# Unrepentant-Atheist/AC-3-ACM-Codec

Measured on AMD Instinct MI355X. Metric: AC-3 5.1@48kHz frames/sec/GPU (decode+encode); achieved HBM GB/s vs peak, higher is better.
Workload: dtype f32+i32

## Files before the change

ac-3-acm-codec_amd/csrc/decode.hip:

```cpp
#include "decode_kernel.h"

namespace ac3mi {

__global__ void lfsr_prefix_kernel(const uint32_t *draws, uint16_t *frame_lfsr, uint32_t *frame_pos, uint16_t *lfsr_state, const int32_t *slot,
                                   const uint16_t *seq, const uint16_t *idx, int n_streams, int frames)
{
    const int s = blockIdx.x * blockDim.x + threadIdx.x;
    if (s >= n_streams) return;
    uint32_t state = lfsr_state[slot ? slot[s] : s];
    uint32_t pos = idx[state];
    for (int f = 0; f < frames; f++) {
        if (frame_pos) frame_pos[(size_t)s * frames + f] = state ? pos : 0xffffffffu;
        else frame_lfsr[(size_t)s * frames + f] = (uint16_t)state;
        const uint32_t k = draws[(size_t)s * frames + f];
        if (state != 0 && k) { pos = (pos + k) % 65535u; state = seq[pos]; }
    }
    if (frame_pos) lfsr_state[slot ? slot[s] : s] = (uint16_t)state;
}

struct MantLDS {
    uint4 dsc[M2_NDESC];
    float qtab[760];
    uint8_t ring[6][M2_LDS_WAVE];
    uint8_t cplbnd[6][20];
};

#ifndef MANT_LB
#define MANT_LB 7
#endif
__global__ __launch_bounds__(384, MANT_LB) void mant_kernel(const MantParams P)
{
    __shared__ MantLDS L;
    extern __shared__ uint32_t frw[];
    const int tid = threadIdx.x, lane = tid & 63;
    const int blk = __builtin_amdgcn_readfirstlane(tid >> 6);
    const unsigned fidx = xcd_remap(blockIdx.x, gridDim.x);
    const size_t unit = (size_t)fidx * 6 + blk;
    const uint4 *dq = reinterpret_cast<const uint4 *>(P.desc + unit);
    const BlkWords D{{dq[0], dq[1], dq[2], dq[3], dq[4]}};
    const uint32_t fposv = P.frame_pos[fidx];
    const int nw = (P.frame_bytes + 3) >> 2;
    const auto fw = stage_frame_fetch<384>(P.frames + (size_t)fidx * P.frame_stride, P.frame_bytes, tid);
    const float q0 = P.tab->qtab[tid];
    float q1 = 0.f;
    if (tid < 760 - 384) q1 = P.tab->qtab[384 + tid];
    float *cblk = P.coef + unit * P.n_in * 256;
    MantBlk B;
    B.nf = P.nfchans; B.lfeon = P.lfeon; B.acmod = P.acmod; B.in_lfe = P.lfeon ? 1 : 0;
    const bool failed = D.head(B);
    const uint64_t rve = D.rv_exp(), rvb = D.rv_bap();
    const uint8_t *const rowbase = P.rows + (size_t)fidx * 6 * ROWSET;
    const RowFetch fetch{rowbase, rve, rvb, lane};
    {
        stage_frame_store<384>(frw, fw, P.frame_bytes, tid);
        if (const int own = D.own_bytes()) trim_staged_frame(frw, own, nw, tid, 384);
        if (tid < M2_NDESC) L.dsc[tid] = mant_desc2((uint32_t)tid);
        L.qtab[tid] = q0;
        if (tid < 760 - 384) L.qtab[384 + tid] = q1;
    }
    const int slot0 = seg_slot(0, B.nf, B.chincpl, B.chincpl ? __builtin_ctz(B.chincpl) : 99);
    uint2 first = make_uint2(0u, 0u);
    if (!failed) first = fetch(slot0);
    __syncthreads();
    if (failed) {
        for (int c = 0; c < P.n_in; c++)
            *reinterpret_cast<float4 *>(cblk + (size_t)c * 256 + 4 * lane) = make_float4(0.f, 0.f, 0.f, 0.f);
        return;
    }
    D.ranges(B);
    B.gainv = D.gainv(lane);
    if (B.chincpl && lane < 18) {
        const uint32_t below = D.cplbndstrc() & ((1u << lane) - 1u);
        L.cplbnd[blk][lane] = (uint8_t)(lane - __popc(below));
    }
    const uint32_t fpos = rfl(fposv);
    const bool lfsr_live = fpos != 0xffffffffu;
    const uint32_t i0 = lfsr_live ? (fpos + D.draw_off()) % 65535u : 0u;
    const float *cc = P.cplco + unit * 90;
    mant_block2<256, true>(B, fetch, first, [&](int c, int bnd) { return cc[c * 18 + bnd]; }, L.cplbnd[blk], L.dsc, L.ring[blk], frw, (uint32_t)nw + 2u,
                L.qtab, reinterpret_cast<const int16_t *>(P.lfsr_seq) + 1 + i0, lfsr_live, cblk, D.bitpos(), lane);
}

}

namespace ac3mi {

#ifdef DEC_STAMPS
}
extern "C" __attribute__((visibility("default"))) int ac3mi_debug_dec_cycles(unsigned long long *out8, int reset)
{
    if (hipMemcpyFromSymbol(out8, HIP_SYMBOL(ac3mi::g_dec_cycles), sizeof(unsigned long long) * 8) != hipSuccess) return -1;
    if (reset) { unsigned long long z[8] = {0}; if (hipMemcpyToSymbol(HIP_SYMBOL(ac3mi::g_dec_cycles), z, sizeof z) != hipSuccess) return -1; }
    return 0;
}
namespace ac3mi {
#endif

hipError_t launch_mantx(const DeviceTables &tab, const DecodeLaunch &L, const MantParams &M, const KernelLaunch &k, hipStream_t stream);
void launch_decode0_src(const DecodeParams &P, unsigned n_streams, size_t fr_bytes, hipStream_t stream);

hipError_t decode_params(const DeviceTables &tab, const DecodeLaunch &L, DecodeParams &P)
{
    if (L.frame_bytes > STAGE_MAX_BYTES) return hipErrorInvalidValue;
    const bool split = L.choice.split;
    P.desc = split ? (BlkDesc *)L.ws_desc : nullptr;
    P.rows = split ? L.ws_rows : nullptr;
    P.cplco = split ? L.ws_cplco : nullptr;
    P.frame_pos = split ? L.ws_fpos : nullptr;
    P.frames = L.frames;
    P.coef = L.coef;
    P.blksw = L.blksw;
    P.zs = L.zs;
    P.status = L.status;
    P.lfsr_state = L.lfsr;
    P.slot = L.slot;
    P.tap_exp = L.tap_exp;
    P.tap_bap = L.tap_bap;
    P.lfsr_seq = tab.lfsr_seq;
    P.lfsr_idx = tab.lfsr_idx;
    P.tab = tab.dec;
    P.n_streams = L.n_streams;
    P.frames_per_stream = L.frames_per_stream;
    P.frame_stride = L.frame_stride;
    P.frame_bytes = L.frame_bytes;
    P.req_flags = L.req_flags;
    P.level = L.level;
    P.dynrng_on = L.dynrng_on;
    P.acmod = L.acmod;
    P.lfeon = L.lfeon;
    P.nfchans = sync_nfchans(L.acmod & 7);
    P.n_in = P.nfchans + (L.lfeon ? 1 : 0);
    P.frame_draws = L.frame_draws;
    P.frame_lfsr = L.frame_lfsr;
    P.dyn_out = L.dyn_out;
    P.dyn_in = L.dyn_in;
    P.crc = L.crc;
    if (L.src_dyn) {
        if (L.dynrng_on || L.dyn_out || L.dyn_in) return hipErrorInvalidValue;
        P.src_dyn = L.src_dyn;
    }
    return hipSuccess;
}

template <uint32_t V> constexpr auto decode_variant()
{
    using Fn = void (*)(DecodeParams);
    if constexpr (V == V_SRC) return (Fn) nullptr;
    else return (Fn)decode_kernel<(int)(V & V_NUM), (V & V_FX) != 0, (V & V_SRC) != 0>;
}
template <uint32_t V> struct DecodeVariant { static constexpr auto fn = decode_variant<V>(); };

hipError_t launch_decode(const DeviceTables &tab, const DecodeLaunch &L, hipStream_t stream)
{
    DecodeParams P;
    const hipError_t ep = decode_params(tab, L, P);
    if (ep != hipSuccess) return ep;
    if (L.n_streams <= 0 || L.frames_per_stream <= 0) return hipSuccess;
    const DecChoice &c = L.choice;
    if (c.err || c.wg) return hipErrorInvalidValue;
    static const int lds_pad = getenv("AC3MI_DEC_LDS_PAD") ? atoi(getenv("AC3MI_DEC_LDS_PAD")) : 0;
    static const int mant_pad = getenv("AC3MI_MANT_LDS_PAD") ? atoi(getenv("AC3MI_MANT_LDS_PAD")) : 0;
    const size_t fr_bytes = staged_frame_lds(L.frame_bytes);
    for (int i = 0; i < c.n; i++) {
// ... 42 lines not shown
```

ac-3-acm-codec_amd/csrc/decode_kernel.h:

```cpp
#pragma once
#include "decode_common.h"
#include "mant2.h"

namespace ac3mi {


#ifndef DEC_LB0
#define DEC_LB0 4
#endif
#ifndef DEC_LBP
#define DEC_LBP 5
#endif
#ifdef DEC_STAMPS
__device__ unsigned long long g_dec_cycles[8];
#define DK_DECL() unsigned long long dk_t = 0, dk_acc[6] = {0, 0, 0, 0, 0, 0}
#define DK_T0() dk_t = __builtin_readcyclecounter()
#define DK_LAP(id) do { const unsigned long long t_ = __builtin_readcyclecounter(); dk_acc[id] += t_ - dk_t; dk_t = t_; } while (0)
#define DK_END() do { if (lane == 0) for (int i_ = 0; i_ < 6; i_++) atomicAdd(&g_dec_cycles[i_], dk_acc[i_]); } while (0)
#else
#define DK_DECL() do { } while (0)
#define DK_T0() do { } while (0)
#define DK_LAP(id) do { } while (0)
#define DK_END() do { } while (0)
#endif
// ... 341 lines not shown
                                const int mybai = st.cbai(slot);
                                const int mydeltbae = slot == 5 ? 2 : st.deltbae(slot == 6 ? 5 : slot);
                                const BaCtx c = ba_ctx(st.bai(), mybai, st.csnroffst(), st.halfrate(), L.hth,
                                                       mydeltbae == 2 ? nullptr : L.deltba[slot == 6 ? 5 : slot],
                                                       slot == 6 ? st.cplfleak() << 8 : 0, slot == 6 ? st.cplsleak() << 8 : 0);
                                bit_allocate_finish(L, L.bmask, c, slot == 6 ? st.cplstrtbnd() : 0, start, end, L.exp + row_off(slot), L.bap + row_off(slot), wide, h, lane);
                            }
                        }
#undef AC3MI_SLOT_END
                    }
                    wave_sync();
                }
                if (rd.get(1)) {
                    const int n = rd.get(9);
                    rd.skip(8 * n);
                }
            } while (0);

            if (!FX && P.tap_exp) {
                uint8_t *te = P.tap_exp + (fidx * 6 + blk) * 7 * 256;
                int8_t *tb = P.tap_bap + (fidx * 6 + blk) * 7 * 256;
                for (int c = 0; c < 7; c++)
                    for (int i = lane; i < 256; i += 64) {
                        const bool in = c != 5 || i < LFE_ROW;
                        te[c * 256 + i] = in ? L.exp[row_off(c) + i] : 0;
                        tb[c * 256 + i] = in ? unmap_width(L.bap[row_off(c) + i]) : 0;
                    }
            }

            if (!err) {
                DK_LAP(3);
                a52_downmix_coeff_hd(gain, acm, st.output, st.dynrng, st.clev, st.slev);

                if (!PARSE && st.chincpl && lane < 18) {
                    const uint32_t below = st.cplbndstrc & ((1u << lane) - 1u);
                    L.cplbnd[lane] = (uint8_t)(lane - __popc(below));
                }
                SegBase sb;
                sb.bit = rd.pos();
                sb.r3 = sb.r5 = sb.r11 = sb.draw = 0;
                if constexpr (!PARSE) {
                    MantBlk B;
                    B.nf = nf; B.lfeon = lfeon; B.acmod = acm; B.in_lfe = in_lfe;
                    B.chincpl = st.chincpl; B.dithmask = dithmask; B.rematflg = st.rematflg();
                    B.cplstrtmant = st.cplstrtmant; B.cplendmant = st.cplendmant();
#pragma unroll
                    for (int i = 0; i < 5; i++) { B.endmant[i] = st.endm(i); B.gain[i] = gain[i]; }
                    B.lfe_gain = (st.output & AC3MI_LFE) ? st.dynrng : 0.f;
                    const uint32_t lfsr_i0 = P.lfsr_idx[st.lfsr];
                    const bool lfsr_live = st.lfsr != 0;
                    mant_block<false>(B, [&](int slot) { return (const uint8_t *)L.exp + row_off(slot); },
                                          [&](int slot) { return (const int8_t *)L.bap + row_off(slot); },
                                          [&](int c, int bnd) { return L.cplco[c][bnd]; }, L.cplbnd, L.desc, L.gcode, frw, FB.last,
                                          P.tab->qtab, P.lfsr_seq, lfsr_i0, lfsr_live, cblk, sb, lane);
                    if (lfsr_live && sb.draw) st.lfsr = P.lfsr_seq[(lfsr_i0 + (uint32_t)sb.draw) % 65535u];
                } else {
                    const int cplfirst = st.chincpl ? __builtin_ctz(st.chincpl) : 99;
                    const int nseg = nf + (st.chincpl ? 1 : 0) + (lfeon ? 1 : 0);
                    const int ncpl_dith = __popc(st.chincpl & dithmask);
                    const int k = lane;
                    const int slot_l = st.chincpl ? (k <= cplfirst ? k : k == cplfirst + 1 ? 6 : k - 1 < nf ? k - 1 : 5) : (k < nf ? k : 5);
                    const bool seg_l = k < nseg;
                    const int end_l = (int)((uint32_t)(st.ends >> (8 * slot_l)) & 0xffu);
                    const int start_l = slot_l == 6 ? st.cplstrtmant : 0;
                    const int mult_l = slot_l < 5 ? (dithmask >> slot_l) & 1 : slot_l == 6 ? ncpl_dith : 0;
                    const uint32_t key_l = 0x80000000u | (uint32_t)start_l | ((uint32_t)end_l << 10);
                    uint32_t ca = L.tot[slot_l][0], cb = L.tot[slot_l][1];
                    for (unsigned long long miss = __ballot(seg_l && L.tot[slot_l][2] != key_l); miss; miss &= miss - 1) {
                        const int k0 = __builtin_ctzll(miss);
                        const int s0 = __builtin_amdgcn_readlane(slot_l, k0);
                        const RowTotals T = row_totals(L.bap + row_off(s0), __builtin_amdgcn_readlane(start_l, k0), __builtin_amdgcn_readlane(end_l, k0),
                                                       s0 == 5 ? LFE_ROW / 4 : 64, lane);
                        if (lane == k0) { ca = T.a; cb = T.b; L.tot[s0][0] = T.a; L.tot[s0][1] = T.b; L.tot[s0][2] = key_l; }
                    }
                    {
                        const uint32_t n3 = seg_l ? (ca >> 13) & 511u : 0u, n5 = seg_l ? ca >> 22 : 0u, n11 = seg_l ? cb & 511u : 0u;
                        const uint32_t nz = seg_l ? cb >> 9 : 0u, plain = seg_l ? ca & 0x1fffu : 0u;
                        const uint32_t own35 = n3 | (n5 << 16), p35 = wave_incl_scan_u32(own35) - own35, r11 = wave_incl_scan_u32(n11) - n11;
                        const uint32_t r3 = p35 & 0xffffu, r5 = p35 >> 16;
                        auto div3 = [](uint32_t x) { return (x * 0xaaabu) >> 17; };
                        const uint32_t o3 = div3(r3 + n3 + 2u) - div3(r3 + 2u), o5 = div3(r5 + n5 + 2u) - div3(r5 + 2u);
                        const uint32_t o11 = ((r11 + n11 + 1u) >> 1) - ((r11 + 1u) >> 1);
                        const uint32_t bits_l = plain + 5u * o3 + 7u * (o5 + o11);
                        const uint32_t tot = wave_sum_u32(bits_l | ((nz * (uint32_t)mult_l) << 16));
                        sb.bit += tot & 0xffffu;
                        sb.draw = (int)(tot >> 16);
                    }
                    {
                        uint8_t *rowset = P.rows + (fidx * 6 + blk) * (size_t)ROWSET;
                        const int used = ((1 << nf) - 1) | (lfeon ? 32 : 0) | (st.chincpl ? 64 : 0);
                        const int we = dirty_exp & used, wb = dirty_bap & used;
                        for (int m = we; m; m &= m - 1) {
                            const int s0 = __builtin_ctz(m);
                            if (lane < (s0 == 5 ? LFE_ROW / 4 : 64))
                                *reinterpret_cast<uint32_t *>(rowset + s0 * 512 + 4 * lane) = *reinterpret_cast<const uint32_t *>(L.exp + row_off(s0) + 4 * lane);
                        }
                        for (int m = wb; m; m &= m - 1) {
                            const int s0 = __builtin_ctz(m);
                            if (lane < (s0 == 5 ? LFE_ROW / 4 : 64))
                                *reinterpret_cast<uint32_t *>(rowset + s0 * 512 + 256 + 4 * lane) = *reinterpret_cast<const uint32_t *>(L.bap + row_off(s0) + 4 * lane);
                        }
                        dirty_exp &= ~we;
                        dirty_bap &= ~wb;
                        rv_exp = ((we >> lane) & 1) ? (uint32_t)blk : rv_exp;
                        rv_bap = ((wb >> lane) & 1) ? (uint32_t)blk : rv_bap;
                    }
                    if (st.chincpl) {
                        float *cc = P.cplco + (fidx * 6 + blk) * 90;
                        cc[lane] = (&L.cplco[0][0])[lane];
                        if (lane < 26) cc[64 + lane] = (&L.cplco[0][0])[64 + lane];
                    }
                    {
                        uint8_t *dp = reinterpret_cast<uint8_t *>(P.desc + (fidx * 6 + blk));
                        const uint32_t fl = ((uint32_t)st.chincpl << BLK_CHINCPL) | ((uint32_t)dithmask << BLK_DITH) | ((uint32_t)st.rematflg() << BLK_REMAT);
                        const uint32_t w0 = lane == 0 ? rd.pos() : lane == 1 ? frame_draws : lane == 2 ? fl : st.cplbndstrc;
                        if (lane < 4) reinterpret_cast<uint32_t *>(dp)[lane] = w0;
                        const int em = lane == 5 ? st.cplstrtmant : lane == 7 ? short_bytes : (int)((uint32_t)(st.ends >> (8 * (lane & 7))) & 0xffu);
                        if (lane < 8) reinterpret_cast<uint16_t *>(dp + offsetof(BlkDesc, endmant))[lane] = (uint16_t)em;
                        if (lane < 8) { dp[offsetof(BlkDesc, rv_exp) + lane] = (uint8_t)rv_exp; dp[offsetof(BlkDesc, rv_bap) + lane] = (uint8_t)rv_bap; }
                        const float gl = lane == 0 ? gain[0] : lane == 1 ? gain[1] : lane == 2 ? gain[2] : lane == 3 ? gain[3] : lane == 4 ? gain[4]
                                       : (st.output & AC3MI_LFE) ? st.dynrng : 0.f;
                        const uint32_t w12 = lane < 6 ? __float_as_uint(gl) : (uint32_t)(16 * st.csnroffst() + (st.cbai(0) >> 3));
                        if (lane < 7) reinterpret_cast<uint32_t *>(dp + offsetof(BlkDesc, gain))[lane] = w12;
                    }
                    bd_ok = true;
                }
                rd.seek(sb.bit);
                frame_draws += (uint32_t)sb.draw;
            }

            DK_LAP(4);
            if (err) { status |= 1u << blk; frame_dead = true; }
            if constexpr (PARSE) {
                if ((err || !bd_ok) && lane == 0) {
                    P.desc[fidx * 6 + blk].flags = BLK_FAILED;
                    P.desc[fidx * 6 + blk].src_snr = 0u;
                    P.desc[fidx * 6 + blk].own_bytes = (uint16_t)short_bytes;
                }
            }
            {
                if (err && !PARSE)
                    for (int c = 0; c < n_in; c++)
                        *reinterpret_cast<float4 *>(cblk + (size_t)c * 256 + 4 * lane) = make_float4(0.f, 0.f, 0.f, 0.f);
                if (P.blksw && lane < nfchans)
                    P.blksw[(fidx * 6 + blk) * nfchans + lane] = (uint8_t)(err ? 0 : ((blkswm >> lane) & 1));
            }
            __builtin_amdgcn_fence(__ATOMIC_RELEASE, "wavefront");
            __builtin_amdgcn_wave_barrier();
        }
        DK_LAP(5);
        if (const uint8_t *crcp = crc_verdicts()) {
            const uint32_t cv = crcp[fidx];
            if (!(status & 0x100u) || (cv & 0x40u)) status |= (cv & 3u) << 10;
        }
        if (lane == 0) P.status[fidx] = status | (reuse0 ? 0x200u : 0u);
        if (lane == 0 && P.zs) P.zs[fidx] = (uint8_t)((status & 0x100u) ? 0 : surround_level_is_zero(acm, st.output, st.slev));
        if (MODE == 5 && lane == 0) P.frame_draws[fidx] = frame_draws;
        if (MODE == 4) {
            if (lane == 0) P.frame_pos[fidx] = pos_live ? lfsr_pos : 0xffffffffu;
            lfsr_pos = (lfsr_pos + frame_draws) % 65535u;
        }
    }
    if (MODE == 0 && lane == 0) P.lfsr_state[sslot] = (uint16_t)st.lfsr;
    if (MODE == 4 && lane == 0 && pos_live) P.lfsr_state[sslot] = P.lfsr_seq[lfsr_pos];
    DK_END();
}

}
```

ac-3-acm-codec_amd/csrc/decode_mx.hip:

```cpp
#include <stdlib.h>
#include "mant2.h"
#include "xform_core.h"
#include "ac3mi_internal.h"

namespace ac3mi {

constexpr int MX_PLANE = 256 + 16;
constexpr int MX_WAVE = 6 * EX_GROUP * 8;
constexpr int MX_RING = 6 * MX_PLANE * 4;
constexpr int MX_TILE = 3072;
static_assert(MX_RING + M2_LDS_WAVE <= MX_WAVE && MX_TILE + 256 * 6 * 2 <= MX_WAVE && 48 * 8 * 8 <= MX_TILE, "region layout");

struct MantxParams {
    MantParams m;
    const uint8_t *blksw;
    float *delay;
    const int32_t *slot;
    int delay_stride;
    float *pcm;
    int16_t *pcm16;
    int8_t wslot[6];
    const float2 *tw_long, *tw_short;
    const float *window;
    float bias;
};

struct MantxLDS {
    uint4 dsc[M2_NDESC];
    float qtab[760];
    float2 tw[2][128];
    float win[256];
    uint8_t cplbnd[6][20];
    uint32_t ready[6];
    alignas(16) uint8_t wave[6][MX_WAVE];
};

#ifndef MANTX_LB
#define MANTX_LB 3
#endif
#ifdef MX_STAMPS
__device__ unsigned long long g_mx_cycles[6][8];
#define MX_T0() unsigned long long mx_t = __builtin_readcyclecounter()
#define MX_LAP(id) do { const unsigned long long t_ = __builtin_readcyclecounter(); if (lane == 0) atomicAdd(&g_mx_cycles[blk][id], t_ - mx_t); mx_t = t_; } while (0)
#else
#define MX_T0() do { } while (0)
#define MX_LAP(id) do { } while (0)
#endif
template <bool S16, bool FX = false>
__global__ __launch_bounds__(384, MANTX_LB) void mantx_kernel(const MantxParams Q)
{
    const MantParams &P = Q.m;
    const int n_in = FX ? 6 : P.n_in, nfchans = FX ? 5 : P.nfchans;
    __shared__ MantxLDS L;
    extern __shared__ uint32_t frw[];
    const int tid = threadIdx.x, lane = tid & 63;
    const int blk = __builtin_amdgcn_readfirstlane(tid >> 6);
    MX_T0();
    const unsigned fidx = xcd_remap(blockIdx.x, gridDim.x);
    const size_t unit = (size_t)fidx * 6 + blk;
    const uint4 *dq = reinterpret_cast<const uint4 *>(P.desc + unit);
    const BlkWords D{{dq[0], dq[1], dq[2], dq[3], dq[4]}};
    const uint32_t fposv = P.frame_pos[fidx];
    const int nw = (P.frame_bytes + 3) >> 2;
    static_assert(offsetof(MantxLDS, win) == offsetof(MantxLDS, tw) + sizeof(float2) * 256, "tw and win are one 3-KB stretch");
    const auto fw = stage_frame_fetch<384>(P.frames + (size_t)fidx * P.frame_stride, P.frame_bytes, tid);
    const float q0 = P.tab->qtab[tid];
    float q1 = 0.f;
    if (tid < 760 - 384) q1 = P.tab->qtab[384 + tid];
    const float2 *twsrc = blk < 2 ? Q.tw_long + tid : blk < 4 ? Q.tw_short + (tid - 128) : reinterpret_cast<const float2 *>(Q.window) + (tid - 256);
    const float2 twv = *twsrc;
    uint8_t *const region = L.wave[blk];
    float *const planes = reinterpret_cast<float *>(region);
    MantBlk B;
    B.nf = nfchans; B.lfeon = FX ? 1 : P.lfeon; B.acmod = FX ? 7 : P.acmod; B.in_lfe = FX ? 1 : P.lfeon ? 1 : 0;
    const bool failed = D.head(B);
    const uint64_t rve = failed ? 0ull : D.rv_exp();
    const uint64_t rvb = failed ? 0ull : D.rv_bap();
    const uint8_t *const rowbase = P.rows + (size_t)fidx * 6 * ROWSET;
    const RowFetch fetch{rowbase, rve, rvb, lane};
    __builtin_assume(B.nf >= 1);
    const int slot0 = seg_slot(0, B.nf, B.chincpl, B.chincpl ? __builtin_ctz(B.chincpl) : 99);
    const uint2 first = fetch(slot0);
    {
        stage_frame_store<384>(frw, fw, P.frame_bytes, tid);
        if (const int own = D.own_bytes()) trim_staged_frame(frw, own, nw, tid, 384);
        if (tid < M2_NDESC) L.dsc[tid] = mant_desc2((uint32_t)tid);
        L.qtab[tid] = q0;
        if (tid < 760 - 384) L.qtab[384 + tid] = q1;
        reinterpret_cast<float2 *>(&L.tw[0][0])[tid] = twv;
        if (tid < 6) L.ready[tid] = 0u;
    }
    __syncthreads();
    MX_LAP(0);

    if (failed) {
        for (int c = 0; c < n_in; c++)
            *reinterpret_cast<float4 *>(planes + c * MX_PLANE + 4 * lane) = make_float4(0.f, 0.f, 0.f, 0.f);
    } else {
        D.ranges(B);
        B.gainv = D.gainv(lane);
        if (B.chincpl && lane < 18) {
            const uint32_t below = D.cplbndstrc() & ((1u << lane) - 1u);
            L.cplbnd[blk][lane] = (uint8_t)(lane - __popc(below));
        }
        const uint32_t fpos = rfl(fposv);
        const bool lfsr_live = fpos != 0xffffffffu;
        const uint32_t i0 = lfsr_live ? (fpos + D.draw_off()) % 65535u : 0u;
        const float *cc = P.cplco + unit * 90;
        mant_block2<MX_PLANE, true>(B, fetch, first, [&](int c, int bnd) { return cc[c * 18 + bnd]; }, L.cplbnd[blk], L.dsc, region + MX_RING, frw,
                              (uint32_t)nw + 2u, L.qtab, reinterpret_cast<const int16_t *>(P.lfsr_seq) + 1 + i0, lfsr_live, planes, D.bitpos(), lane);
    }
    wave_sync();

    MX_LAP(1);
    const int l8 = lane & 7, grp = lane >> 3;
    const bool own = grp < n_in;
    const int o = own ? grp : 0;
    const int fb = o - B.in_lfe;
    const bool sw = fb >= 0 && Q.blksw[unit * nfchans + fb] != 0;
    const size_t sidx = Q.slot ? (size_t)Q.slot[fidx] : (size_t)fidx;
    float *const dptr = Q.delay + sidx * Q.delay_stride + (size_t)o * 128;
    float2 dl[8];
    if (blk == 0) {
#pragma unroll
        for (int j = 0; j < 8; j++) {
            const int i = ((j & 1) ? 15 - l8 : l8) + 16 * (j >> 1);
            dl[j] = *reinterpret_cast<const float2 *>(dptr + 2 * i);
        }
    }
    FirstTail ft;
#pragma unroll
    for (int j = 0; j < 8; j++) ft.f0[j] = ft.f1[j] = ft.t0[j] = ft.t1[j] = 0.f;
    {
        const float *plane = planes + o * MX_PLANE;
        float xa[16], xb[16];
        if (!sw) {
            const float2 *p = reinterpret_cast<const float2 *>(plane) + l8;
            float2 v[16];
#pragma unroll
            for (int n = 0; n < 16; n++) v[n] = p[8 * n];
#pragma unroll
            for (int n = 0; n < 16; n++) {
                xa[n] = __builtin_fmaf(1.f, v[n].x, 0.f);
                xb[n] = __builtin_fmaf(1.f, mirror8(v[15 - n].y), 0.f);
            }
        } else {
            const int f = l8 >> 2, n2 = l8 & 3;
            const float *pa = plane + 4 * n2 + f;
            const float *pb = plane + 254 + f - 4 * n2;
#pragma unroll
            for (int n = 0; n < 16; n++) {
                xa[n] = __builtin_fmaf(1.f, pa[16 * n], 0.f);
                xb[n] = __builtin_fmaf(1.f, pb[-16 * n], 0.f);
            }
        }
        wave_sync();
        float2 *ex = reinterpret_cast<float2 *>(region) + o * EX_GROUP;
        const float2 *tw = &L.tw[sw ? 1 : 0][l8 * 16];
        cf r[16];
        imdct_first_half(xa, xb, tw, ex, l8, r);
        if (!sw) imdct_long_second_half(r, ft);
        else imdct_short_second_half(r, ft);
    }
    __builtin_amdgcn_fence(__ATOMIC_RELEASE, "wavefront");
    __builtin_amdgcn_wave_barrier();
    if (blk < 5 && lane < 48) {
        float2 *tl = reinterpret_cast<float2 *>(region);
#pragma unroll
        for (int j = 0; j < 8; j++) tl[j * 48 + lane] = make_float2(ft.t0[j], ft.t1[j]);
    }
    MX_LAP(2);
    if (blk == 0) asm volatile("s_waitcnt vmcnt(0)" ::: "memory");
    if (blk < 5) __hip_atomic_store(&L.ready[blk], 1u, __ATOMIC_RELEASE, __HIP_MEMORY_SCOPE_WORKGROUP);
    if (blk > 0) {
        for (int spin = 0; spin < (1 << 20) && __hip_atomic_load(&L.ready[blk - 1], __ATOMIC_ACQUIRE, __HIP_MEMORY_SCOPE_WORKGROUP) == 0u; spin++)
            __builtin_amdgcn_s_sleep(1);
        const float2 *tl = reinterpret_cast<const float2 *>(L.wave[blk - 1]);
        const int ls = lane < 48 ? lane : l8;
#pragma unroll
        for (int j = 0; j < 8; j++) dl[j] = tl[j * 48 + ls];
    }
    if (blk == 5) {
        for (int spin = 0; spin < (1 << 20) && __hip_atomic_load(&L.ready[0], __ATOMIC_ACQUIRE, __HIP_MEMORY_SCOPE_WORKGROUP) == 0u; spin++)
            __builtin_amdgcn_s_sleep(1);
    }
    if (blk == 5 && own) {
#pragma unroll
        for (int j = 0; j < 8; j++) {
            const int i = ((j & 1) ? 15 - l8 : l8) + 16 * (j >> 1);
            *reinterpret_cast<float2 *>(dptr + 2 * i) = make_float2(ft.t0[j], ft.t1[j]);
        }
    }

// ... 91 lines not shown
```

ac-3-acm-codec_amd/csrc/mant2.h:

```cpp
#pragma once
#include "decode_common.h"

namespace ac3mi {

constexpr int M2_RING = 3 * 128;
constexpr int M2_LDS_WAVE = M2_RING + 256;
constexpr int M2_NDESC = 97;
constexpr int LFSR_EXT = 16384;


struct alignas(16) BlkDesc {
    uint32_t bitpos;
    uint32_t draw_off;
    uint32_t flags;
    uint32_t cplbndstrc;
    uint16_t endmant[5], cplstrt, cplend;
    uint16_t own_bytes;
    uint8_t rv_exp[8], rv_bap[8];
    float gain[5], lfe_gain;
    uint32_t src_snr;
    uint32_t pad1;
};
constexpr uint32_t BLK_FAILED = 1u;
constexpr int BLK_CHINCPL = 8, BLK_DITH = 16, BLK_REMAT = 24;
static_assert(sizeof(BlkDesc) == BLKDESC_BYTES && offsetof(BlkDesc, src_snr) == BLKDESC_SRC_SNR, "what the host sizes and reads (ac3mi_internal.h)");

constexpr int ROWSET = 7 * 512;

static_assert(offsetof(BlkDesc, bitpos) == 0 && offsetof(BlkDesc, draw_off) == 4 && offsetof(BlkDesc, flags) == 8 && offsetof(BlkDesc, cplbndstrc) == 12,
              "lanes 0-3: the first four dwords");
static_assert(offsetof(BlkDesc, cplstrt) == offsetof(BlkDesc, endmant) + 2 * 5 && offsetof(BlkDesc, cplend) == offsetof(BlkDesc, endmant) + 2 * 6 &&
              offsetof(BlkDesc, own_bytes) == offsetof(BlkDesc, endmant) + 2 * 7, "lanes 0-7: eight halfwords from endmant on; 6 = the coupling slot");
static_assert(offsetof(BlkDesc, lfe_gain) == offsetof(BlkDesc, gain) + 4 * 5 && offsetof(BlkDesc, src_snr) == offsetof(BlkDesc, gain) + 4 * 6,
              "lanes 0-6: seven dwords from gain on");

struct BlkWords {
    uint4 q[sizeof(BlkDesc) / 16];
    template <size_t OFF> __device__ __forceinline__ uint32_t u32() const
    {
        static_assert(OFF % 4 == 0 && OFF < sizeof(BlkDesc), "a dword of the descriptor");
        constexpr int j = (OFF / 4) & 3;
        const uint4 &v = q[OFF / 16];
        return j == 0 ? v.x : j == 1 ? v.y : j == 2 ? v.z : v.w;
    }
    template <size_t OFF> __device__ __forceinline__ uint32_t s32() const { return rfl(u32<OFF>()); }
    template <size_t OFF> __device__ __forceinline__ uint32_t s16() const
    {
        static_assert(OFF % 2 == 0, "a halfword of the descriptor");
        return (s32<OFF & ~(size_t)3>() >> (8 * (OFF & 3))) & 0xffffu;
    }
    __device__ __forceinline__ bool head(MantBlk &B) const
    {
        const uint32_t flags = s32<offsetof(BlkDesc, flags)>();
        B.chincpl = (int)((flags >> BLK_CHINCPL) & 31u); B.dithmask = (int)((flags >> BLK_DITH) & 31u); B.rematflg = (int)((flags >> BLK_REMAT) & 15u);
        return (flags & BLK_FAILED) != 0u;
    }
    __device__ __forceinline__ void ranges(MantBlk &B) const
    {
        constexpr size_t E = offsetof(BlkDesc, endmant);
        B.cplstrtmant = (int)s16<offsetof(BlkDesc, cplstrt)>(); B.cplendmant = (int)s16<offsetof(BlkDesc, cplend)>();
        B.ends = (uint64_t)((s16<E>() & 0xffu) | ((s16<E + 2>() & 0xffu) << 8) | ((s16<E + 4>() & 0xffu) << 16) | ((s16<E + 6>() & 0xffu) << 24)) |
                 ((uint64_t)(s16<E + 8>() & 0xffu) << 32);
    }
    __device__ __forceinline__ float gainv(int lane) const
    {
        constexpr size_t G = offsetof(BlkDesc, gain);
        return __uint_as_float(lane == 0 ? u32<G>() : lane == 1 ? u32<G + 4>() : lane == 2 ? u32<G + 8>() : lane == 3 ? u32<G + 12>()
                             : lane == 4 ? u32<G + 16>() : u32<offsetof(BlkDesc, lfe_gain)>());
    }
    __device__ __forceinline__ int own_bytes() const { return (int)s16<offsetof(BlkDesc, own_bytes)>(); }
    __device__ __forceinline__ uint32_t cplbndstrc() const { return s32<offsetof(BlkDesc, cplbndstrc)>(); }
    __device__ __forceinline__ uint32_t bitpos() const { return s32<offsetof(BlkDesc, bitpos)>(); }
    __device__ __forceinline__ uint32_t draw_off() const { return s32<offsetof(BlkDesc, draw_off)>(); }
    __device__ __forceinline__ uint64_t rv_exp() const { return (uint64_t)s32<offsetof(BlkDesc, rv_exp)>() | ((uint64_t)s32<offsetof(BlkDesc, rv_exp) + 4>() << 32); }
    __device__ __forceinline__ uint64_t rv_bap() const { return (uint64_t)s32<offsetof(BlkDesc, rv_bap)>() | ((uint64_t)s32<offsetof(BlkDesc, rv_bap) + 4>() << 32); }
};

struct RowFetch {
    const uint8_t *const &rowbase;
    const uint64_t &rve, &rvb;
    const int &lane;
    __device__ __forceinline__ uint2 operator()(int slot) const
    {
        const uint8_t *er = rowbase + (size_t)((rve >> (8 * slot)) & 7u) * ROWSET + slot * 512;
        const uint8_t *br = rowbase + (size_t)((rvb >> (8 * slot)) & 7u) * ROWSET + slot * 512 + 256;
        if (slot == 5) return lane < 7 ? make_uint2(br[lane], er[lane]) : make_uint2(1u, 0u);
        return make_uint2(reinterpret_cast<const uint32_t *>(br)[lane], reinterpret_cast<const uint32_t *>(er)[lane]);
    }
};

__host__ __device__ inline uint4 mant_desc2(uint32_t b)
{
    const uint32_t k1 = b >> 5, nbp = b >= 32 ? 0u : b == 1 ? 0u : b;
    const uint32_t inc = k1 == 1 ? 1u << 20 : k1 == 2 ? 1u << 10 : k1 == 3 ? 1u : 0u;
    const uint32_t obits = k1 == 1 ? 5u : k1 ? 7u : 0u, per = k1 == 3 ? 2u : k1 ? 3u : 0u, sh = 30u - 10u * k1;
    const uint32_t recip = k1 == 3 ? 1024u : k1 ? 683u : 0u;
    const uint32_t qbase = k1 == 1 ? 0u : k1 == 2 ? 96u : k1 == 3 ? 480u : nbp == 3 ? 736u : nbp == 4 ? 744u : 0u;
    const uint32_t coded = (k1 || nbp == 3 || nbp == 4) ? 1u : 0u, zero = b == 0 ? 1u : 0u;
    const uint32_t ring = k1 ? 128u * (k1 - 1u) : 0u;
    return make_uint4(inc, nbp | (obits << 8) | (per << 16) | (sh << 24), recip | (qbase << 16), ring | (zero << 16) | (coded << 24));
}

struct MantParams {
    const uint8_t *frames;
    const BlkDesc *desc;
    const uint8_t *rows;
    const float *cplco;
    const uint32_t *frame_pos;
    float *coef;
    const uint16_t *lfsr_seq;
    const DecTables *tab;
    unsigned n_frames;
    int frame_stride, frame_bytes;
    int acmod, lfeon, n_in, nfchans;
};

struct Seg2 {
    uint32_t bit;
    uint32_t phase;
    uint32_t draw;
};

template <int NB>
struct Bins2 {
    uint32_t raw[NB];
    uint32_t rs[NB];
    uint32_t dy[NB], dz[NB], dw[NB];
    uint32_t cd;
};

template <int NB>
__device__ __forceinline__ void seg2_first(uint32_t bytes4, const uint4 *dsc, uint8_t *ring, const uint32_t *frw, uint32_t frw_last,
                                           int mult, Seg2 &S, Bins2<NB> &R, int lane)
{
    uint32_t inc[NB], gl = 0;
#pragma unroll
    for (int j = 0; j < NB; j++) {
        const uint32_t b = (bytes4 >> (8 * j)) & 0xffu;
        const uint4 d = dsc[b];
        inc[j] = d.x; R.dy[j] = d.y; R.dz[j] = d.z; R.dw[j] = d.w;
        gl += d.x;
    }
    const uint32_t gin = wave_incl_scan_u32(gl);
    uint32_t run = gin - gl + S.phase;
    uint32_t nb[NB], nbsum = 0, ndsum = 0, slot[NB];
#pragma unroll
    for (int j = 0; j < NB; j++) {
        const uint32_t x = __builtin_amdgcn_ubfe(run, R.dy[j] >> 24, 10);
        run += inc[j];
        const uint32_t q = (x * (R.dz[j] & 0xffffu)) >> 11;
        const uint32_t mem = x - q * ((R.dy[j] >> 16) & 0xffu);
        const uint32_t ob = mem == 0u ? (R.dy[j] >> 8) & 0xffu : 0u;
        nb[j] = (R.dy[j] & 0xffu) + ob;
        nbsum += nb[j];
        ndsum += ((R.dw[j] >> 16) & 0xffu) * (uint32_t)mult;
        const uint32_t rslot = (R.dw[j] & 0xffffu) + (q & 127u);
        R.rs[j] = rslot | (mem << 16);
        slot[j] = ob != 0u ? rslot : (uint32_t)(M2_RING + 4 * lane);
    }
    const uint32_t bl = nbsum | (ndsum << 16);
    const uint32_t bin_ = wave_incl_scan_u32(bl);
    const uint32_t gtot = wave_last(gin), btot = wave_last(bin_);
    R.cd = S.draw + (bin_ >> 16) - ndsum;
    const uint32_t off = S.bit + (bin_ & 0xffffu) - nbsum;
    uint32_t wi = off >> 5;
    wi = wi < frw_last ? wi : frw_last;
    const uint32_t d0 = frw[wi], d1 = frw[wi + 1], d2 = frw[wi + 2];
    const uint32_t k = off & 31u;
    uint64_t win = ((((uint64_t)d0 << 32) | d1) << k) | (uint64_t)((d2 >> 1) >> (31u - k));
#pragma unroll
    for (int j = 0; j < NB; j++) {
        R.raw[j] = ((uint32_t)(win >> 32) >> 1) >> (31u - nb[j]);
        win <<= nb[j];
        ring[slot[j]] = (uint8_t)R.raw[j];
    }
    S.bit += btot & 0xffffu;
    S.draw += btot >> 16;
    {
        const uint32_t x3 = ((S.phase >> 20) & 1023u) + ((gtot >> 20) & 1023u), x5 = ((S.phase >> 10) & 1023u) + ((gtot >> 10) & 1023u),
                       x11 = (S.phase & 1023u) + (gtot & 1023u);
        const uint32_t q3 = (x3 * 683u) >> 11, q5 = (x5 * 683u) >> 11, q11 = x11 >> 1;
        S.phase = (((q3 & 127u) * 3u + (x3 - 3u * q3)) << 20) | (((q5 & 127u) * 3u + (x5 - 3u * q5)) << 10) | ((q11 & 127u) * 2u + (x11 & 1u));
    }
}

template <int NB>
__device__ __forceinline__ void seg2_values(const Bins2<NB> &R, const uint8_t *ring, const float *qtab, float *q)
{
    uint32_t code[NB];
#pragma unroll
    for (int j = 0; j < NB; j++) code[j] = ring[R.rs[j] & 0xffffu];
#pragma unroll
    for (int j = 0; j < NB; j++) { asm volatile("" : "+v"(code[j])); code[j] &= 0xffu; }
    float tv[NB];
#pragma unroll
    for (int j = 0; j < NB; j++) {
        const uint32_t per = (R.dy[j] >> 16) & 0xffu;
        const uint32_t sel = per ? code[j] * per + (R.rs[j] >> 16) : R.raw[j];
        tv[j] = qtab[(R.dw[j] >> 24) ? (R.dz[j] >> 16) + sel : 0u];
    }
#pragma unroll
    for (int j = 0; j < NB; j++) {
        const uint32_t nbp = R.dy[j] & 0xffu;
        const float pv = (float)(((int32_t)(R.raw[j] << ((32u - nbp) & 31u))) >> 16);
        q[j] = (R.dw[j] >> 24) ? tv[j] : pv;
    }
}

__device__ __forceinline__ float dither2(const int16_t *seq, uint32_t i) { return (float)((3 * (int)seq[i]) >> 2); }

template <int PS = 256, bool PK = false, class Fetch, class Cplco>
__device__ __forceinline__ void mant_block2(const MantBlk &B, Fetch fetch, uint2 first, Cplco cplco_of, const uint8_t *cplbnd, const uint4 *dsc, uint8_t *ring,
                                            const uint32_t *frw, uint32_t frw_last, const float *qtab, const int16_t *seq1, bool lfsr_live,
                                            float *cblk, uint32_t bitpos, int lane)
{
    const int nf = B.nf;
    const int ncpl_dith = __popc(B.chincpl & B.dithmask);
    const int em0 = PK ? (int)((uint32_t)B.ends & 0xffu) : B.endmant[0], em1 = PK ? (int)(((uint32_t)B.ends >> 8) & 0xffu) : B.endmant[1];
    const int remat_end = em0 < em1 ? em0 : em1;
    const bool remat_late = B.acmod == 2 && B.rematflg != 0 && B.chincpl != 0 && remat_end > B.cplstrtmant;
    const int cplfirst = B.chincpl ? __builtin_ctz(B.chincpl) : 99;
    const int nseg = nf + (B.chincpl ? 1 : 0) + (B.lfeon ? 1 : 0);
    Seg2 S;
    S.bit = bitpos;
    S.phase = 0;
    S.draw = 0;
    uint2 nxt = first;
    for (int k = 0; k < nseg; k++) {
        const int slot = seg_slot(k, nf, B.chincpl, cplfirst);
        const uint2 cur = nxt;
        if (k + 1 < nseg) nxt = fetch(seg_slot(k + 1, nf, B.chincpl, cplfirst));
        if (slot == 5) {
            Bins2<1> R;
            seg2_first<1>(lane < 7 ? cur.x & 0xffu : 1u, dsc, ring, frw, frw_last, 0, S, R, lane);
            wave_sync();
            float q;
            seg2_values<1>(R, ring, qtab, &q);
            const float lfe_gain = PK ? __builtin_bit_cast(float, __builtin_amdgcn_readlane(__builtin_bit_cast(int, B.gainv), 5)) : B.lfe_gain;
            const float v = q * (sf_of((int)(cur.y & 0xffu)) * lfe_gain);
            const float z = 0.f * (sf_of(0) * lfe_gain);
            if (lane < 8) cblk[lane] = lane < 7 ? v : z;
            if (lane >= 2) *reinterpret_cast<float4 *>(cblk + 4 * lane) = make_float4(z, z, z, z);
            continue;
        }
        int start = 0, end, draws;
        float g = 0.f;
        if (slot < 5) {
            if (PK) {
                end = (int)((uint32_t)(B.ends >> (8 * slot)) & 0xffu);
                g = __builtin_bit_cast(float, __builtin_amdgcn_readlane(__builtin_bit_cast(int, B.gainv), slot));
            } else {
                end = slot == 0 ? B.endmant[0] : slot == 1 ? B.endmant[1] : slot == 2 ? B.endmant[2] : slot == 3 ? B.endmant[3] : B.endmant[4];
                g = slot == 0 ? B.gain[0] : slot == 1 ? B.gain[1] : slot == 2 ? B.gain[2] : slot == 3 ? B.gain[3] : B.gain[4];
            }
            draws = (B.dithmask >> slot) & 1;
        } else {
            start = B.cplstrtmant;
            end = B.cplendmant;
            draws = ncpl_dith;
        }
        uint32_t bytes4;
        {
            int lo = start - 4 * lane, hi = end - 4 * lane;
            lo = lo < 0 ? 0 : lo > 4 ? 4 : lo;
            hi = hi < 0 ? 0 : hi > 4 ? 4 : hi;
            const uint32_t below_hi = (uint32_t)((1ull << (8 * hi)) - 1ull), below_lo = (uint32_t)((1ull << (8 * lo)) - 1ull);
            const uint32_t m = below_hi & ~below_lo;
            bytes4 = (cur.x & m) | (0x01010101u & ~m);
        }
        Bins2<4> R;
        seg2_first<4>(bytes4, dsc, ring, frw, frw_last, draws, S, R, lane);
        wave_sync();
        if (slot < 5) {
            float out[4], qv[4];
            seg2_values<4>(R, ring, qtab, qv);
            const bool dith = draws != 0 && lfsr_live;
            const uint32_t z0 = (R.dw[0] >> 16) & 0xffu, z1 = (R.dw[1] >> 16) & 0xffu, z2 = (R.dw[2] >> 16) & 0xffu, z3 = (R.dw[3] >> 16) & 0xffu;
            if (dith && __any((z0 | z1 | z2 | z3) != 0u)) {
                const int16_t *sp = seq1 + R.cd;
                const float d0 = dither2(sp, 0), d1 = dither2(sp, z0), d2 = dither2(sp, z0 + z1), d3 = dither2(sp, z0 + z1 + z2);
                qv[0] = z0 ? d0 : qv[0]; qv[1] = z1 ? d1 : qv[1]; qv[2] = z2 ? d2 : qv[2]; qv[3] = z3 ? d3 : qv[3];
            }
#pragma unroll
            for (int j = 0; j < 4; j++) {
                const int e = (int)((cur.y >> (8 * j)) & 0xffu);
                out[j] = qv[j] * (sf_of(e) * g);
            }
            float *plane = cblk + (slot + B.in_lfe) * PS;
            if (slot == 1 && B.acmod == 2 && B.rematflg != 0 && !remat_late) {
                float4 a4 = *reinterpret_cast<const float4 *>(plane - PS + 4 * lane);
                float a[4] = {a4.x, a4.y, a4.z, a4.w};
#pragma unroll
                for (int j = 0; j < 4; j++) {
                    const int bin = 4 * lane + j;
                    const int band = bin < 25 ? 0 : bin < 37 ? 1 : bin < 61 ? 2 : 3;
                    if (bin >= 13 && (bin < remat_end || (bin == 13 && remat_end <= 13)) && ((B.rematflg >> band) & 1)) {
                        const float x = a[j], v = out[j];
                        a[j] = x + v;
                        out[j] = x - v;
                    }
                }
                *reinterpret_cast<float4 *>(plane - PS + 4 * lane) = make_float4(a[0], a[1], a[2], a[3]);
            }
            if ((B.chincpl >> slot) & 1) {
#pragma unroll
                for (int j = 0; j < 4; j++) {
                    const int bin = 4 * lane + j;
                    if (bin < end || bin < B.cplstrtmant || bin >= B.cplendmant) plane[bin] = bin >= B.cplendmant ? 0.f : out[j];
                }
            } else {
                *reinterpret_cast<float4 *>(plane + 4 * lane) = make_float4(out[0], out[1], out[2], out[3]);
            }
        } else {
            uint32_t cd = R.cd;
            float qv[4];
            seg2_values<4>(R, ring, qtab, qv);
#pragma unroll
            for (int j = 0; j < 4; j++) {
                const int bin = 4 * lane + j;
                const bool in = bin >= start && bin < end;
                const bool zero = ((R.dw[j] >> 16) & 0xffu) != 0u;
                const int e = (int)((cur.y >> (8 * j)) & 0xffu);
                const float m = qv[j] * sf_of(e);
                const int bnd = cplbnd[in ? (bin - start) / 12 : 0];
                uint32_t cdc = cd;
                for (int c = 0; c < nf; c++) {
                    if (!((B.chincpl >> c) & 1)) continue;
                    const float gc = PK ? __builtin_bit_cast(float, __builtin_amdgcn_readlane(__builtin_bit_cast(int, B.gainv), c))
                                        : c == 0 ? B.gain[0] : c == 1 ? B.gain[1] : c == 2 ? B.gain[2] : c == 3 ? B.gain[3] : B.gain[4];
                    const float co = cplco_of(c, bnd) * gc;
                    float v = m * co;
                    if (zero) {
                        v = 0.f;
                        if ((B.dithmask >> c) & 1) { v = (sf_of(e) * co) * (lfsr_live ? dither2(seq1, cdc) : 0.f); cdc++; }
                    }
                    if (in) cblk[(c + B.in_lfe) * PS + bin] = v;
                }
                cd += zero ? (uint32_t)draws : 0u;
            }
        }
    }
    if (remat_late) {
        wave_sync();
        volatile float *p0 = cblk + (size_t)B.in_lfe * PS, *p1 = p0 + PS;
        for (int bin = 13 + lane; bin < remat_end; bin += 64) {
            const int band = bin < 25 ? 0 : bin < 37 ? 1 : bin < 61 ? 2 : 3;
            if ((B.rematflg >> band) & 1) {
                const float a = p0[bin], v = p1[bin];
                p0[bin] = a + v;
                p1[bin] = a - v;
            }
        }
    }
}

}
```

Measured before the change: 9.565 million.

## Precompute per-segment start bits/phase in decode pass and ride LFE on last segment

The earlier decode pass now writes each segment's starting bit offset, dither-draw count and grouping phase into spare rowset bytes through an inclusive wave scan. The mantissa kernel reads these start words back, so segments no longer depend on running totals carried from the previous segment. The end-of-segment scan and phase arithmetic in seg2_first are dropped. The LFE segment is also folded into the last full-bandwidth segment when that channel's bins end early enough, which saves one segment pass. In exchange the decode kernel does extra global stores, the mantissa kernel does an extra load, and the lane-masking logic becomes more complex.

```diff
diff --git a/ac-3-acm-codec_amd/csrc/decode.hip b/ac-3-acm-codec_amd/csrc/decode.hip
--- a/ac-3-acm-codec_amd/csrc/decode.hip
+++ b/ac-3-acm-codec_amd/csrc/decode.hip
@@ -39,6 +39,7 @@
     const uint4 *dq = reinterpret_cast<const uint4 *>(P.desc + unit);
     const BlkWords D{{dq[0], dq[1], dq[2], dq[3], dq[4]}};
     const uint32_t fposv = P.frame_pos[fidx];
+    const SegWords segw = SegWords::fetch(P.rows + unit * ROWSET, lane);
     const int nw = (P.frame_bytes + 3) >> 2;
     const auto fw = stage_frame_fetch<384>(P.frames + (size_t)fidx * P.frame_stride, P.frame_bytes, tid);
     const float q0 = P.tab->qtab[tid];
@@ -78,7 +79,7 @@
     const uint32_t i0 = lfsr_live ? (fpos + D.draw_off()) % 65535u : 0u;
     const float *cc = P.cplco + unit * 90;
     mant_block2<256, true>(B, fetch, first, [&](int c, int bnd) { return cc[c * 18 + bnd]; }, L.cplbnd[blk], L.dsc, L.ring[blk], frw, (uint32_t)nw + 2u,
-                L.qtab, reinterpret_cast<const int16_t *>(P.lfsr_seq) + 1 + i0, lfsr_live, cblk, D.bitpos(), lane);
+                L.qtab, reinterpret_cast<const int16_t *>(P.lfsr_seq) + 1 + i0, lfsr_live, cblk, D.bitpos(), segw, lane);
 }
 
 }
diff --git a/ac-3-acm-codec_amd/csrc/decode_kernel.h b/ac-3-acm-codec_amd/csrc/decode_kernel.h
--- a/ac-3-acm-codec_amd/csrc/decode_kernel.h
+++ b/ac-3-acm-codec_amd/csrc/decode_kernel.h
@@ -447,9 +447,15 @@
                         const uint32_t o3 = div3(r3 + n3 + 2u) - div3(r3 + 2u), o5 = div3(r5 + n5 + 2u) - div3(r5 + 2u);
                         const uint32_t o11 = ((r11 + n11 + 1u) >> 1) - ((r11 + 1u) >> 1);
                         const uint32_t bits_l = plain + 5u * o3 + 7u * (o5 + o11);
-                        const uint32_t tot = wave_sum_u32(bits_l | ((nz * (uint32_t)mult_l) << 16));
-                        sb.bit += tot & 0xffffu;
-                        sb.draw = (int)(tot >> 16);
+                        const uint32_t own = seg_start_word(bits_l, nz * (uint32_t)mult_l), upto = wave_incl_scan_u32(own), tot = wave_last(upto);
+                        sb.bit += seg_start_bits(tot);
+                        sb.draw = (int)seg_start_draws(tot);
+                        uint8_t *segs = P.rows + (fidx * 6 + blk) * (size_t)ROWSET + SEG_WORDS_OFF;
+                        if (seg_l) *reinterpret_cast<uint2 *>(segs + 8 * k) = make_uint2(upto - own, seg_phase_word(r3, r5, r11));
+                        if (lane < 4)
+                            *reinterpret_cast<uint32_t *>(segs + (SEG_LFE_OFF - SEG_WORDS_OFF) + 4 * lane) =
+                                seg_lfe_dword(*reinterpret_cast<const uint16_t *>(L.bap + row_off(5) + 2 * lane),
+                                              *reinterpret_cast<const uint16_t *>(L.exp + row_off(5) + 2 * lane));
                     }
                     {
                         uint8_t *rowset = P.rows + (fidx * 6 + blk) * (size_t)ROWSET;
diff --git a/ac-3-acm-codec_amd/csrc/decode_mx.hip b/ac-3-acm-codec_amd/csrc/decode_mx.hip
--- a/ac-3-acm-codec_amd/csrc/decode_mx.hip
+++ b/ac-3-acm-codec_amd/csrc/decode_mx.hip
@@ -61,6 +61,7 @@
     const uint4 *dq = reinterpret_cast<const uint4 *>(P.desc + unit);
     const BlkWords D{{dq[0], dq[1], dq[2], dq[3], dq[4]}};
     const uint32_t fposv = P.frame_pos[fidx];
+    const SegWords segw = SegWords::fetch(P.rows + unit * ROWSET, lane);
     const int nw = (P.frame_bytes + 3) >> 2;
     static_assert(offsetof(MantxLDS, win) == offsetof(MantxLDS, tw) + sizeof(float2) * 256, "tw and win are one 3-KB stretch");
     const auto fw = stage_frame_fetch<384>(P.frames + (size_t)fidx * P.frame_stride, P.frame_bytes, tid);
@@ -108,7 +109,7 @@
         const uint32_t i0 = lfsr_live ? (fpos + D.draw_off()) % 65535u : 0u;
         const float *cc = P.cplco + unit * 90;
         mant_block2<MX_PLANE, true>(B, fetch, first, [&](int c, int bnd) { return cc[c * 18 + bnd]; }, L.cplbnd[blk], L.dsc, region + MX_RING, frw,
-                              (uint32_t)nw + 2u, L.qtab, reinterpret_cast<const int16_t *>(P.lfsr_seq) + 1 + i0, lfsr_live, planes, D.bitpos(), lane);
+                              (uint32_t)nw + 2u, L.qtab, reinterpret_cast<const int16_t *>(P.lfsr_seq) + 1 + i0, lfsr_live, planes, D.bitpos(), segw, lane);
     }
     wave_sync();
 
diff --git a/ac-3-acm-codec_amd/csrc/mant2.h b/ac-3-acm-codec_amd/csrc/mant2.h
--- a/ac-3-acm-codec_amd/csrc/mant2.h
+++ b/ac-3-acm-codec_amd/csrc/mant2.h
@@ -1,5 +1,6 @@
 #pragma once
 #include "decode_common.h"
+#include "seg_start.h"
 
 namespace ac3mi {
 
@@ -26,6 +27,28 @@
 static_assert(sizeof(BlkDesc) == BLKDESC_BYTES && offsetof(BlkDesc, src_snr) == BLKDESC_SRC_SNR, "what the host sizes and reads (ac3mi_internal.h)");
 
 constexpr int ROWSET = 7 * 512;
+constexpr int SEG_WORDS_OFF = 5 * 512 + 128, SEG_LFE_OFF = SEG_WORDS_OFF + 8 * (SEG_MAX + 1);
+static_assert(SEG_WORDS_OFF % 8 == 0 && SEG_WORDS_OFF >= 5 * 512 + LFE_ROW && SEG_LFE_OFF + 16 <= 5 * 512 + 256,
+              "past the LFE's row, inside the half (SegWords::fetch reads eight pairs and four dwords)");
+__host__ __device__ inline uint32_t seg_lfe_dword(uint32_t rowbytes2, uint32_t exps2)
+{
+    return (rowbytes2 & 0xffu) | ((exps2 & 0xffu) << 8) | ((rowbytes2 & 0xff00u) << 8) | ((exps2 & 0xff00u) << 16);
+}
+
+constexpr int LFE_RIDE_LANE = 56, LFE_RIDE_END = 4 * LFE_RIDE_LANE;
+static_assert(LFE_RIDE_LANE + 7 <= 64 && LFE_RIDE_LANE % 8 == 0, "seven lanes; LFE bin = the lane's low three bits");
+
+struct SegWords {
+    uint32_t v;
+    static __device__ __forceinline__ SegWords fetch(const uint8_t *rowset, int lane)
+    {
+        const int i = lane < 16 ? 2 * (lane & 7) + ((lane >> 3) & 1) : (SEG_LFE_OFF - SEG_WORDS_OFF) / 4 + ((lane >> 1) & 3);
+        return SegWords{reinterpret_cast<const uint32_t *>(rowset + SEG_WORDS_OFF)[i]};
+    }
+    __device__ __forceinline__ uint32_t w0(int k) const { return (uint32_t)__builtin_amdgcn_readlane((int)v, k); }
+    __device__ __forceinline__ uint32_t w1(int k) const { return (uint32_t)__builtin_amdgcn_readlane((int)v, k + 8); }
+    __device__ __forceinline__ uint32_t lfe_bin(int lane) const { return (v >> (16 * (lane & 1))) & 0xffffu; }
+};
 
 static_assert(offsetof(BlkDesc, bitpos) == 0 && offsetof(BlkDesc, draw_off) == 4 && offsetof(BlkDesc, flags) == 8 && offsetof(BlkDesc, cplbndstrc) == 12,
               "lanes 0-3: the first four dwords");
@@ -131,14 +154,14 @@
 
 template <int NB>
 __device__ __forceinline__ void seg2_first(uint32_t bytes4, const uint4 *dsc, uint8_t *ring, const uint32_t *frw, uint32_t frw_last,
-                                           int mult, Seg2 &S, Bins2<NB> &R, int lane)
+                                           int mult, const Seg2 &S, Bins2<NB> &R, int lane, uint32_t keep0 = ~0u)
 {
     uint32_t inc[NB], gl = 0;
 #pragma unroll
     for (int j = 0; j < NB; j++) {
         const uint32_t b = (bytes4 >> (8 * j)) & 0xffu;
         const uint4 d = dsc[b];
-        inc[j] = d.x; R.dy[j] = d.y; R.dz[j] = d.z; R.dw[j] = d.w;
+        inc[j] = d.x; R.dy[j] = d.y; R.dz[j] = d.z; R.dw[j] = j == 0 ? d.w & keep0 : d.w;
         gl += d.x;
     }
     const uint32_t gin = wave_incl_scan_u32(gl);
@@ -160,7 +183,6 @@
     }
     const uint32_t bl = nbsum | (ndsum << 16);
     const uint32_t bin_ = wave_incl_scan_u32(bl);
-    const uint32_t gtot = wave_last(gin), btot = wave_last(bin_);
     R.cd = S.draw + (bin_ >> 16) - ndsum;
     const uint32_t off = S.bit + (bin_ & 0xffffu) - nbsum;
     uint32_t wi = off >> 5;
@@ -174,14 +196,6 @@
         win <<= nb[j];
         ring[slot[j]] = (uint8_t)R.raw[j];
     }
-    S.bit += btot & 0xffffu;
-    S.draw += btot >> 16;
-    {
-        const uint32_t x3 = ((S.phase >> 20) & 1023u) + ((gtot >> 20) & 1023u), x5 = ((S.phase >> 10) & 1023u) + ((gtot >> 10) & 1023u),
-                       x11 = (S.phase & 1023u) + (gtot & 1023u);
-        const uint32_t q3 = (x3 * 683u) >> 11, q5 = (x5 * 683u) >> 11, q11 = x11 >> 1;
-        S.phase = (((q3 & 127u) * 3u + (x3 - 3u * q3)) << 20) | (((q5 & 127u) * 3u + (x5 - 3u * q5)) << 10) | ((q11 & 127u) * 2u + (x11 & 1u));
-    }
 }
 
 template <int NB>
@@ -212,7 +226,7 @@
 template <int PS = 256, bool PK = false, class Fetch, class Cplco>
 __device__ __forceinline__ void mant_block2(const MantBlk &B, Fetch fetch, uint2 first, Cplco cplco_of, const uint8_t *cplbnd, const uint4 *dsc, uint8_t *ring,
                                             const uint32_t *frw, uint32_t frw_last, const float *qtab, const int16_t *seq1, bool lfsr_live,
-                                            float *cblk, uint32_t bitpos, int lane)
+                                            float *cblk, uint32_t bitpos, SegWords segw, int lane)
 {
     const int nf = B.nf;
     const int ncpl_dith = __popc(B.chincpl & B.dithmask);
@@ -221,15 +235,25 @@
     const bool remat_late = B.acmod == 2 && B.rematflg != 0 && B.chincpl != 0 && remat_end > B.cplstrtmant;
     const int cplfirst = B.chincpl ? __builtin_ctz(B.chincpl) : 99;
     const int nseg = nf + (B.chincpl ? 1 : 0) + (B.lfeon ? 1 : 0);
-    Seg2 S;
-    S.bit = bitpos;
-    S.phase = 0;
-    S.draw = 0;
+    auto end_of = [&](int slot) {
+        if (PK) return (int)((uint32_t)(B.ends >> (8 * slot)) & 0xffu);
+        return slot == 0 ? B.endmant[0] : slot == 1 ? B.endmant[1] : slot == 2 ? B.endmant[2] : slot == 3 ? B.endmant[3] : B.endmant[4];
+    };
+    bool ride = false;
+    if (B.lfeon && nseg >= 2) {
+        const int before = seg_slot(nseg - 2, nf, B.chincpl, cplfirst);
+        if (before < 5) ride = end_of(before) <= LFE_RIDE_END;
+    }
+    const int npass = ride ? nseg - 1 : nseg;
+    const bool lfe_lane = lane >= LFE_RIDE_LANE && lane < LFE_RIDE_LANE + 7;
     uint2 nxt = first;
-    for (int k = 0; k < nseg; k++) {
+    for (int k = 0; k < npass; k++) {
         const int slot = seg_slot(k, nf, B.chincpl, cplfirst);
         const uint2 cur = nxt;
-        if (k + 1 < nseg) nxt = fetch(seg_slot(k + 1, nf, B.chincpl, cplfirst));
+        const uint32_t w0 = segw.w0(k);
+        const Seg2 S{bitpos + seg_start_bits(w0), segw.w1(k), seg_start_draws(w0)};
+        const bool riding = ride && k == npass - 1;
+        if (k + 1 < npass) nxt = fetch(seg_slot(k + 1, nf, B.chincpl, cplfirst));
         if (slot == 5) {
             Bins2<1> R;
             seg2_first<1>(lane < 7 ? cur.x & 0xffu : 1u, dsc, ring, frw, frw_last, 0, S, R, lane);
@@ -246,13 +270,9 @@
         int start = 0, end, draws;
         float g = 0.f;
         if (slot < 5) {
-            if (PK) {
-                end = (int)((uint32_t)(B.ends >> (8 * slot)) & 0xffu);
-                g = __builtin_bit_cast(float, __builtin_amdgcn_readlane(__builtin_bit_cast(int, B.gainv), slot));
-            } else {
-                end = slot == 0 ? B.endmant[0] : slot == 1 ? B.endmant[1] : slot == 2 ? B.endmant[2] : slot == 3 ? B.endmant[3] : B.endmant[4];
-                g = slot == 0 ? B.gain[0] : slot == 1 ? B.gain[1] : slot == 2 ? B.gain[2] : slot == 3 ? B.gain[3] : B.gain[4];
-            }
+            end = end_of(slot);
+            if (PK) g = __builtin_bit_cast(float, __builtin_amdgcn_readlane(__builtin_bit_cast(int, B.gainv), slot));
+            else g = slot == 0 ? B.gain[0] : slot == 1 ? B.gain[1] : slot == 2 ? B.gain[2] : slot == 3 ? B.gain[3] : B.gain[4];
             draws = (B.dithmask >> slot) & 1;
         } else {
             start = B.cplstrtmant;
@@ -268,12 +288,22 @@
             const uint32_t m = below_hi & ~below_lo;
             bytes4 = (cur.x & m) | (0x01010101u & ~m);
         }
+        const bool lfe_bin = riding && lfe_lane;
+        if (lfe_bin) bytes4 = (segw.lfe_bin(lane) & 0xffu) | 0x01010100u;
         Bins2<4> R;
-        seg2_first<4>(bytes4, dsc, ring, frw, frw_last, draws, S, R, lane);
+        seg2_first<4>(bytes4, dsc, ring, frw, frw_last, draws, S, R, lane, lfe_bin ? ~0x00ff0000u : ~0u);
         wave_sync();
         if (slot < 5) {
             float out[4], qv[4];
             seg2_values<4>(R, ring, qtab, qv);
+            if (riding) {
+                const float lfe_gain = PK ? __builtin_bit_cast(float, __builtin_amdgcn_readlane(__builtin_bit_cast(int, B.gainv), 5)) : B.lfe_gain;
+                const float v = qv[0] * (sf_of((int)(segw.lfe_bin(lane) >> 8)) * lfe_gain);
+                const float z = 0.f * (sf_of(0) * lfe_gain);
+                if (lane >= LFE_RIDE_LANE) cblk[lane - LFE_RIDE_LANE] = lfe_lane ? v : z;
+                if (lane >= 2) *reinterpret_cast<float4 *>(cblk + 4 * lane) = make_float4(z, z, z, z);
+                if (lfe_lane) qv[0] = 0.f;
+            }
             const bool dith = draws != 0 && lfsr_live;
             const uint32_t z0 = (R.dw[0] >> 16) & 0xffu, z1 = (R.dw[1] >> 16) & 0xffu, z2 = (R.dw[2] >> 16) & 0xffu, z3 = (R.dw[3] >> 16) & 0xffu;
             if (dith && __any((z0 | z1 | z2 | z3) != 0u)) {
diff --git a/ac-3-acm-codec_amd/csrc/seg_start.h b/ac-3-acm-codec_amd/csrc/seg_start.h
--- /dev/null
+++ b/ac-3-acm-codec_amd/csrc/seg_start.h
@@ -0,0 +1,35 @@
+#pragma once
+#include <stdint.h>
+
+#ifndef __HIPCC__
+#ifndef __host__
+#define __host__
+#endif
+#ifndef __device__
+#define __device__
+#endif
+#endif
+
+namespace ac3mi {
+
+constexpr uint32_t SEG_RING_SLOTS = 128;
+constexpr int SEG_MAX = 7;
+
+__host__ __device__ inline uint32_t seg_phase_field(uint32_t r, uint32_t members)
+{
+    return members == 2u ? r & (2u * SEG_RING_SLOTS - 1u) : r - 3u * SEG_RING_SLOTS * ((r * 0xaaabu) >> 24);
+}
+
+__host__ __device__ inline uint32_t seg_phase_word(uint32_t r3, uint32_t r5, uint32_t r11)
+{
+    return (seg_phase_field(r3, 3u) << 20) | (seg_phase_field(r5, 3u) << 10) | seg_phase_field(r11, 2u);
+}
+
+constexpr uint32_t SEG_BLOCK_MAX_BINS = 5 * 253 + 216 + 7;
+constexpr uint32_t SEG_BLOCK_MAX_BITS = SEG_BLOCK_MAX_BINS * 16, SEG_BLOCK_MAX_DRAWS = 5 * 253 + 5 * 216;
+static_assert(SEG_BLOCK_MAX_BITS < (1u << 16) && SEG_BLOCK_MAX_DRAWS < (1u << 16), "word 0's halves");
+__host__ __device__ inline uint32_t seg_start_word(uint32_t bits_before, uint32_t draws_before) { return bits_before | (draws_before << 16); }
+__host__ __device__ inline uint32_t seg_start_bits(uint32_t w0) { return w0 & 0xffffu; }
+__host__ __device__ inline uint32_t seg_start_draws(uint32_t w0) { return w0 >> 16; }
+
+}
```

Measured after the change: 9.659 million (median of 6 runs). About the same (+1.0%).
